# Atarilab/iterative_learning_NMPC

Hardware: AMD Instinct MI355X
Metric: MPC solves/sec (horizon-50 centroidal, batch) (higher is better)
Workload: dtype f32; 1 GPU; configs[1]: batch=1024/GPU centroidal quadruped NMPC nx=12 nu=12 N=50 fp32, 1 SQP x 6 IPM Riccati sweeps per solve, warm-start shift + solve per step; global_batch=1024, horizon=50, parallelism=dp1 (independent problems; no collective)

## Files before the change

include/nmpc.h:

```cpp
#ifndef NMPC_H
#define NMPC_H
#include <stddef.h>

#ifdef __cplusplus
extern "C" {
#endif

#define NMPC_MODEL_DOUBLE_INTEGRATOR 0
#define NMPC_MODEL_CENTROIDAL        1
#define NMPC_MODEL_WHOLEBODY         2

#define NMPC_MP_DT    0
#define NMPC_MP_MASS  1
#define NMPC_MP_IXX   2
#define NMPC_MP_IYY   3
#define NMPC_MP_IZZ   4
#define NMPC_MP_GZ    5
#define NMPC_MP_MU    6
#define NMPC_MP_UMAX  7
#define NMPC_MP_PGAIN 8
#define NMPC_MP_HIPX  9
#define NMPC_MP_HIPY  10
#define NMPC_MP_LHIP  11
#define NMPC_MP_L1    12
// ... 41 lines not shown
int nmpc_shift_warm_start(void *handle, int B, int shift, float *X, float *U, void *stream);

int nmpc_solve_batch(void *handle, int B, const float *x0, const float *yref, int yref_per_stage,
                     const float *yref_e, const float *params, float *X, float *U, int *status,
                     float *stats, void *stream);

int nmpc_shift_solve_batch(void *handle, int B, int shift, const float *x0, const float *yref,
                           int yref_per_stage, const float *yref_e, const float *params, float *X,
                           float *U, int *status, float *stats, void *stream);

int nmpc_riccati_batch(void *handle, int Bsz, int nx, int nu, const float *Q, const float *R,
                       const float *q, const float *r, const float *A, const float *B_,
                       const float *d, const float *dx0, float *dX, float *dU, int *status,
                       void *stream);

int nmpc_tracking_error(void *handle, int B, int T, int ns, const float *S, const float *S_nom,
                        float *err, float *weight, float threshold, float ood_weight, void *stream);

typedef struct {
    int n_replans;
    int nodes_per_replan;
    int replanning_steps;
    int nodes_per_cycle;
    int start_node;
    int first_solve;
    int max_sqp_first;
    float nlp_tol_first;
    float nlp_tol;
    double sim_dt, time_horizon, nom_height, height_offset;
    float push_start, push_duration;
    int footsteps;
    int record_sim_steps;
    float hip_offset[8];
    float stance_ratio[4];
    float nominal_period;
    float foot_size;
    int terminate_mask;
    float collision_height;
} nmpc_rollout_cfg;
#define NMPC_ROLLOUT_FLAG_SOLVER        1
#define NMPC_ROLLOUT_FLAG_ROLL          2
#define NMPC_ROLLOUT_FLAG_PITCH         4
#define NMPC_ROLLOUT_FLAG_HEIGHT        8
#define NMPC_ROLLOUT_FLAG_VEL_TRACKING 16
#define NMPC_ROLLOUT_FLAG_COLLISION    32
#define NMPC_ROLLOUT_FLAG_MASK       0xFF
#define NMPC_ROLLOUT_TERM_SHIFT         8
int nmpc_rollout_batch(void *handle, int B, const nmpc_rollout_cfg *cfg, const signed char *gait, float *x,
                       const double *v_des, const double *w_des, double *ref_state, float *foot_pos,
                       const float *push_force, const float *phase, float *X, float *U, float *S,
                       int *status, int *failed, void *stream);

#define NMPC_ROLLOUT_FLAG_JOINT_LIMIT   64

typedef struct {
    int n_replans;
    int replanning_steps;
    int nodes_per_cycle;
    int first_solve;
    int last_node;
    int max_sqp_first;
    float nlp_tol_first;
    float nlp_tol;
    double sim_dt, time_horizon, nom_height, height_offset;
    float step_height;
    float push_start, push_duration;
    int record_sim_steps;
    int force_reference_gravity;
    float nominal_period;
    int terminate_mask;
    float collision_height;
} nmpc_wb_rollout_cfg;
int nmpc_wb_rollout_batch(void *handle, int B, const nmpc_wb_rollout_cfg *cfg, const signed char *gait,
                          const signed char *peaks, const int *nodes, float *q, float *v, const double *v_des,
                          const double *w_des, double *ref_state, const float *joint_ref, const float *push_force,
                          float *X, float *U, float *S, int *status, int *failed, void *stream);

int nmpc_wb_rollout_set_actions(void *handle, void *torque_handle, const int *zoh, float kp, float kd, float *A);

int nmpc_set_skip(void *handle, const int *flags, int mask);

int nmpc_debug_read_tile(void *handle, int b, int k, int which, float *out_host);

int nmpc_debug_read_workspace(void *handle, int b, size_t offset, size_t count, float *out_host);
int nmpc_debug_wb_layout(int N, size_t *out8);

int nmpc_debug_set_buffer(void *handle, float *dev_buffer);

#ifdef __cplusplus
}
#endif
#endif
```

iterative_learning_nmpc_amd/_lib.py:

```python
from __future__ import annotations

import ctypes
import os
from ctypes import POINTER, c_char_p, c_float, c_int, c_size_t, c_void_p
from typing import Optional

import torch

_HERE = os.path.dirname(os.path.abspath(__file__))
LIB_PATH = os.environ.get("NMPC_HIP_LIB") or os.path.join(_HERE, "libnmpc_hip.so")

NMPC_OK = 0
NMPC_STATUS_OK, NMPC_STATUS_NAN, NMPC_STATUS_MAXITER, NMPC_STATUS_MINSTEP, NMPC_STATUS_QP = 0, 1, 2, 3, 4
STATUS_NAMES = {NMPC_STATUS_OK: "ok", NMPC_STATUS_NAN: "nan", NMPC_STATUS_MAXITER: "max_iter",
                NMPC_STATUS_MINSTEP: "min_step", NMPC_STATUS_QP: "qp_failure"}
NMPC_ROLLOUT_FLAG_SOLVER = 1
NMPC_ROLLOUT_FLAG_ROLL = 2
NMPC_ROLLOUT_FLAG_PITCH = 4
NMPC_ROLLOUT_FLAG_HEIGHT = 8
NMPC_ROLLOUT_FLAG_VEL_TRACKING = 16
NMPC_ROLLOUT_FLAG_COLLISION = 32
NMPC_ROLLOUT_FLAG_JOINT_LIMIT = 64
NMPC_ROLLOUT_FLAG_MASK = 0xFF
NMPC_ROLLOUT_TERM_SHIFT = 8

SIGNATURES = {
    "nmpc_model_dims": (c_int, [c_int, POINTER(c_int), POINTER(c_int), POINTER(c_int), POINTER(c_int)]),
    "nmpc_model_output_dims": (c_int, [c_int, POINTER(c_int), POINTER(c_int)]),
    "nmpc_create": (c_int, [c_void_p, c_int, POINTER(c_void_p)]),
    "nmpc_destroy": (None, [c_void_p]),
    "nmpc_last_error": (c_char_p, [c_void_p]),
    "nmpc_workspace_bytes": (c_size_t, [c_void_p]),
    "nmpc_set_model_params": (c_int, [c_void_p, POINTER(c_float), c_int]),
    "nmpc_set_weights": (c_int, [c_void_p, POINTER(c_float), POINTER(c_float), c_float, c_float]),
    "nmpc_set_opts": (c_int, [c_void_p, c_int, c_int, c_float, c_float, c_int]),
    "nmpc_set_contact_patterns": (c_int, [c_void_p, c_int]),
    "nmpc_set_skip": (c_int, [c_void_p, c_void_p, c_int]),
    "nmpc_wb_rollout_set_actions": (c_int, [c_void_p, c_void_p, c_void_p, c_float, c_float, c_void_p]),
    "nmpc_set_ipm": (c_int, [c_void_p, c_float, c_float, c_float, c_float, c_float, c_float]),
    "nmpc_shift_warm_start": (c_int, [c_void_p, c_int, c_int, c_void_p, c_void_p, c_void_p]),
    "nmpc_solve_batch": (c_int, [c_void_p, c_int, c_void_p, c_void_p, c_int, c_void_p, c_void_p,
                                 c_void_p, c_void_p, c_void_p, c_void_p, c_void_p]),
    "nmpc_shift_solve_batch": (c_int, [c_void_p, c_int, c_int, c_void_p, c_void_p, c_int, c_void_p, c_void_p,
                                 c_void_p, c_void_p, c_void_p, c_void_p, c_void_p]),
    "nmpc_riccati_batch": (c_int, [c_void_p, c_int, c_int, c_int] + [c_void_p] * 12),
    "nmpc_tracking_error": (c_int, [c_void_p, c_int, c_int, c_int, c_void_p, c_void_p, c_void_p,
                                    c_void_p, c_float, c_float, c_void_p]),
    "nmpc_rollout_batch": (c_int, [c_void_p, c_int, c_void_p] + [c_void_p] * 14),
    "nmpc_wb_rollout_batch": (c_int, [c_void_p, c_int, c_void_p] + [c_void_p] * 16),
    "nmpc_policy_create": (c_int, [c_void_p, c_int, POINTER(c_void_p)]),
    "nmpc_policy_destroy": (None, [c_void_p]),
    "nmpc_policy_last_error": (ctypes.c_char_p, [c_void_p]),
    "nmpc_policy_param_count": (ctypes.c_size_t, [c_void_p]),
    "nmpc_policy_set_params": (c_int, [c_void_p, c_void_p, c_void_p, c_void_p, c_void_p]),
    "nmpc_policy_get_params": (c_int, [c_void_p, c_void_p, c_void_p, c_void_p, c_void_p]),
    "nmpc_policy_forward": (c_int, [c_void_p, c_int, c_void_p, c_void_p, c_void_p]),
    "nmpc_policy_train_step": (c_int, [c_void_p, c_int, c_void_p, c_void_p, c_float, c_void_p, c_void_p, c_void_p]),
    "nmpc_weighted_sample": (c_int, [c_void_p, ctypes.c_longlong, c_int, ctypes.c_ulonglong, c_void_p, c_void_p, c_void_p]),
    "nmpc_gather_rows": (c_int, [c_void_p, ctypes.c_longlong, c_int, c_void_p, c_int, c_void_p, c_void_p]),
    "nmpc_policy_train_epoch_scratch": (ctypes.c_size_t, [ctypes.c_longlong]),
    "nmpc_policy_train_epoch": (c_int, [c_void_p, c_void_p, c_void_p, c_int, c_int, ctypes.c_ulonglong, c_float, c_void_p,
                                        c_void_p, c_void_p, c_void_p]),
    "nmpc_policy_loss": (c_int, [c_void_p, ctypes.c_longlong, c_void_p, c_void_p, c_void_p, c_void_p]),
    "nmpc_dataset_last_error": (ctypes.c_char_p, []),
    "nmpc_ring_append": (c_int, [c_void_p, c_int, ctypes.c_longlong, c_void_p, ctypes.c_longlong, ctypes.c_longlong, c_void_p]),
    "nmpc_column_stats_scratch": (ctypes.c_size_t, [c_int]),
    "nmpc_column_stats": (c_int, [c_void_p, ctypes.c_longlong, c_int, c_void_p, c_void_p, c_void_p, c_void_p]),
    "nmpc_assemble_batch": (c_int, [c_void_p, c_int, c_void_p, c_void_p, c_int, c_void_p, c_int, c_void_p, c_void_p,
                                    c_void_p, c_int, ctypes.c_longlong, c_void_p, c_int, c_void_p, c_void_p, c_void_p]),
    "nmpc_torque_create": (c_int, [c_void_p, c_int, POINTER(c_void_p)]),
    "nmpc_torque_destroy": (None, [c_void_p]),
    "nmpc_torque_last_error": (ctypes.c_char_p, [c_void_p]),
    "nmpc_id_torques_batch": (c_int, [c_void_p, c_int, c_void_p, c_void_p, c_void_p, c_void_p, c_void_p, c_void_p]),
    "nmpc_pd_torques_batch": (c_int, [c_void_p, c_int, c_void_p, c_void_p, c_void_p, c_void_p, c_void_p, c_float, c_float,
                                      c_void_p, c_void_p]),
    "nmpc_pd_target_action_batch": (c_int, [c_void_p, c_int, c_void_p, c_void_p, c_void_p, c_void_p, c_float, c_float,
                                            c_void_p, c_void_p]),
    "nmpc_plan_actions_batch": (c_int, [c_void_p, c_int, c_int, c_int, c_void_p, c_void_p, c_void_p, ctypes.c_double,
                                        ctypes.c_double, c_float, c_float, c_void_p, c_void_p, c_int, c_void_p, c_int, c_void_p]),
    "nmpc_debug_read_tile": (c_int, [c_void_p, c_int, c_int, c_int, POINTER(c_float)]),
    "nmpc_debug_set_buffer": (c_int, [c_void_p, c_void_p]),
    "nmpc_debug_read_workspace": (c_int, [c_void_p, c_int, c_size_t, c_size_t, POINTER(c_float)]),
    "nmpc_debug_wb_layout": (c_int, [c_int, POINTER(c_size_t)]),
}


class NmpcPolicyDims(ctypes.Structure):
    _fields_ = [("n_in", c_int), ("n_out", c_int), ("n_hidden", c_int), ("hidden", c_int),
                ("batch_norm", c_int), ("batch_max", c_int)]


class NmpcBatchSource(ctypes.Structure):
    _fields_ = [("states", c_void_p), ("n_state", c_int), ("s_mean", c_void_p), ("s_std", c_void_p), ("s_first", c_int),
                ("goals", c_void_p), ("n_goal", c_int), ("g_mean", c_void_p), ("g_std", c_void_p),
                ("actions", c_void_p), ("n_action", c_int), ("n_rows", ctypes.c_longlong)]


class NmpcTreeModel(ctypes.Structure):
    _fields_ = [("n_joints", c_int), ("n_actuated", c_int), ("n_feet", c_int),
                ("parent", POINTER(c_int)), ("type", POINTER(c_int)), ("axis", POINTER(c_float)),
                ("placement", POINTER(c_float)), ("mass", POINTER(c_float)), ("com", POINTER(c_float)),
                ("inertia", POINTER(c_float)), ("foot_joint", POINTER(c_int)), ("foot_offset", POINTER(c_float)),
                ("gravity", c_float * 3)]


class NmpcRolloutCfg(ctypes.Structure):
    _fields_ = [("n_replans", c_int), ("nodes_per_replan", c_int), ("replanning_steps", c_int),
                ("nodes_per_cycle", c_int), ("start_node", c_int), ("first_solve", c_int),
                ("max_sqp_first", c_int), ("nlp_tol_first", c_float), ("nlp_tol", c_float),
                ("sim_dt", ctypes.c_double), ("time_horizon", ctypes.c_double), ("nom_height", ctypes.c_double),
                ("height_offset", ctypes.c_double), ("push_start", c_float), ("push_duration", c_float),
                ("footsteps", c_int), ("record_sim_steps", c_int), ("hip_offset", c_float * 8),
                ("stance_ratio", c_float * 4), ("nominal_period", c_float), ("foot_size", c_float),
                ("terminate_mask", c_int), ("collision_height", c_float)]


class NmpcWbRolloutCfg(ctypes.Structure):
    _fields_ = [("n_replans", c_int), ("replanning_steps", c_int), ("nodes_per_cycle", c_int), ("first_solve", c_int),
                ("last_node", c_int), ("max_sqp_first", c_int), ("nlp_tol_first", c_float), ("nlp_tol", c_float),
                ("sim_dt", ctypes.c_double), ("time_horizon", ctypes.c_double), ("nom_height", ctypes.c_double),
                ("height_offset", ctypes.c_double), ("step_height", c_float), ("push_start", c_float), ("push_duration", c_float),
                ("record_sim_steps", c_int), ("force_reference_gravity", c_int), ("nominal_period", c_float),
                ("terminate_mask", c_int), ("collision_height", c_float)]


class NmpcDims(ctypes.Structure):
    _fields_ = [("model_id", c_int), ("N", c_int), ("B_max", c_int), ("precision", c_int)]


_lib = None


def load() -> ctypes.CDLL:
    global _lib
    if _lib is not None:
        return _lib
    if not os.path.exists(LIB_PATH):
        raise ImportError(
            f"{LIB_PATH} not found: build the HIP extension first "
            "(python -c 'import __graft_entry__ as g; g.build()' or iterative_learning_nmpc_amd/csrc/build.sh). "
            "This package has no CPU fallback.")
    try:
        lib = ctypes.CDLL(LIB_PATH)
    except OSError as e:
        raise ImportError(f"cannot load {LIB_PATH}: {e}") from e
    for name, (res, args) in SIGNATURES.items():
        fn = getattr(lib, name)
        fn.restype, fn.argtypes = res, args
    _lib = lib
    return lib


class NmpcError(RuntimeError):
    pass


_LAST_ERROR = {"solve": "nmpc_last_error", "policy": "nmpc_policy_last_error", "torque": "nmpc_torque_last_error",
               "dataset": "nmpc_dataset_last_error"}


def check(rc: int, handle=None, what: str = "", family: str = "solve") -> None:
    if rc != NMPC_OK:
        last_error = getattr(load(), _LAST_ERROR[family])
        msg = last_error() if family == "dataset" else last_error(handle)
        raise NmpcError(f"{what} failed ({rc}): {msg.decode() if msg else ''}")

# ... 8 lines not shown
```

iterative_learning_nmpc_amd/csrc/nmpc_api.hip:

```cpp
#include <hip/hip_runtime.h>

#include <cmath>
#include <cstdio>
#include <cstdlib>
#include <cstring>
#include <string>

#include "../../include/nmpc_torque.h"
#include "nmpc_host.hpp"
#include "nmpc_torque_plan.hpp"
#include "nmpc_solve.hip"
#include "nmpc_wb.hip"
#include "nmpc_aux.hip.inc"
#include "nmpc_rollout.hip.inc"
#include "nmpc_wb_rollout.hip.inc"

namespace {

using nmpc::fail;
using nmpc::launched;

struct Handle {
    nmpc_dims dims{};
    int device = 0;
// ... 50 lines not shown
nmpc::SolveArgs base_args(const Handle* h) {
    nmpc::SolveArgs a = handle_args<nmpc::SolveArgs>(h);
    for (int j = 0; j < 16; ++j)
        a.rs_free[j] = (j < h->nu) ? 1.0f / std::sqrt(h->W[h->nx + j] + h->reg) : 1.0f;
    a.line_search = h->line_search; a.rho = h->rho;
    a.dbg = h->dbg;
    return a;
}

template <class M>
size_t ws_floats_per_problem(int N) { return nmpc::WsLayout<M>(N).stride; }

nmpc::wb::WbArgs wb_args(const Handle* h) {
    nmpc::wb::WbArgs a = handle_args<nmpc::wb::WbArgs>(h);
    a.precision = h->dims.precision;
    a.pos_rows = h->pos_rows ? 1 : 0;
    return a;
}

int clean_workspace(Handle* h, hipStream_t st) {
    if (h->ws_dirty) {
        NMPC_TRY(h, hipMemsetAsync(h->ws, 0, h->ws_bytes, st));
        h->ws_dirty = false;
    }
    return NMPC_OK;
}

template <class A>
int launch_sqp(Handle* h, A a, hipStream_t st, size_t lds_bytes, void (*qp)(const A), void (*linearize)(const A)) {
    if (lds_bytes > 64 * 1024)
        NMPC_TRY(h, hipFuncSetAttribute(reinterpret_cast<const void*>(qp), hipFuncAttributeMaxDynamicSharedMemorySize, (int)lds_bytes));
    const long long nthreads = (long long)a.B * (a.N + 1);
    const unsigned lin_blocks = (unsigned)((nthreads + 63) / 64);
    const int shift = a.shift;
    for (int it = 0; it < a.max_sqp; ++it) {
        a.it = it;
        a.shift = (it == 0) ? shift : 0;
        if (linearize) hipLaunchKernelGGL(linearize, dim3(lin_blocks), dim3(64), 0, st, a);
        hipLaunchKernelGGL(qp, dim3(a.B), dim3(64), lds_bytes, st, a);
    }
    return launched(h);
}

int launch_wb(Handle* h, nmpc::wb::WbArgs a, hipStream_t st) {
    if (h->line_search) return fail(h, NMPC_E_ARG, "the whole-body model takes full steps (line_search = 0)");
    auto misaligned = [](const void* p, unsigned m) { return (reinterpret_cast<uintptr_t>(p) & (m - 1u)) != 0; };
    if (misaligned(a.x0, 8) || misaligned(a.yref, 8) || misaligned(a.yref_e, 8) || misaligned(a.X, 8) || misaligned(a.U, 8) || misaligned(a.params, 16))
        return fail(h, NMPC_E_ARG, "whole-body arrays must be 8 B aligned (params: 16 B)");
    return launch_sqp(h, a, st, (size_t)nmpc::wb::WbLds(a.N).total * sizeof(float), nmpc::wb::nmpc_wb_qp_kernel,
                      nmpc::wb::nmpc_wb_linearize_kernel);
}

template <class M, bool LEAN, bool BF16B, bool ALLV>
int launch_qp(Handle* h, nmpc::SolveArgs a, hipStream_t st) {
    const size_t bytes = (size_t)nmpc::Lds<M, LEAN>(a.N).total * sizeof(float);
    if (bytes > 160 * 1024) return fail(h, NMPC_E_ARG, "horizon too long for the LDS-resident layout");
    void (*const qp)(const nmpc::SolveArgs) = nmpc::nmpc_qp_kernel<M, LEAN, BF16B, ALLV>;
    void (*const linearize)(const nmpc::SolveArgs) = nmpc::nmpc_linearize_kernel<M>;
    return launch_sqp(h, a, st, bytes, qp, nmpc::qp_linearizes_itself(LEAN, a.N) ? nullptr : linearize);
}

template <class M>
int launch_solve(Handle* h, nmpc::SolveArgs a, hipStream_t st) {
    if (a.N > 64 * nmpc::N_LANE_STAGES) return fail(h, NMPC_E_ARG, "horizon too long for the lane = stage phases");
    auto in_flight = [&](size_t lds_bytes, long long per_simd) -> long long {
        if (lds_bytes > 160 * 1024) return 0;
        const long long by_lds = (long long)((160 * 1024) / lds_bytes);
        return (long long)h->n_cu * (by_lds < 4 * per_simd ? by_lds : 4 * per_simd);
    };
    const long long resident_waves = in_flight((size_t)nmpc::Lds<M, false>(a.N).total * sizeof(float), 1);
    const long long lean_waves = in_flight((size_t)nmpc::Lds<M, true>(a.N).total * sizeof(float), 2);
    const bool lean = h->force_variant ? (h->force_variant > 1)
                                       : (resident_waves == 0 || ((long long)a.B > resident_waves && lean_waves > resident_waves));
    if constexpr (M::N_STATIC_MASKS > 4) {
        if (h->all_patterns) {
            if (h->dims.precision == 1)
                return lean ? launch_qp<M, true, true, true>(h, a, st) : launch_qp<M, false, true, true>(h, a, st);
            return lean ? launch_qp<M, true, false, true>(h, a, st) : launch_qp<M, false, false, true>(h, a, st);
        }
    }
    if (h->dims.precision == 1)
        return lean ? launch_qp<M, true, true, false>(h, a, st) : launch_qp<M, false, true, false>(h, a, st);
    return lean ? launch_qp<M, true, false, false>(h, a, st) : launch_qp<M, false, false, false>(h, a, st);
}

template <class M>
int read_tile(Handle* h, int b, int k, int which, float* out) {
    using G = nmpc::TileGeom<M>;
    const nmpc::WsLayout<M> wl(h->dims.N);
    const size_t off[4] = {wl.At + (size_t)k * G::A_FLOATS, wl.Bt + (size_t)k * G::B_FLOATS,
                           wl.Kt + (size_t)k * G::K_FLOATS, wl.Ct + (size_t)k * G::C_FLOATS};
    const size_t len[4] = {G::A_FLOATS, G::B_FLOATS, G::K_FLOATS, G::C_FLOATS};
    float img[512];
    NMPC_TRY(h, hipMemcpy(img, h->ws + (size_t)b * wl.stride + off[which], len[which] * sizeof(float),
                         hipMemcpyDeviceToHost));
    std::memset(out, 0, 256 * sizeof(float));
    if (which == 0) {
        for (int c = 0; c <= M::NX; ++c)
            for (int i = 0; i < M::NX; ++i) out[i * 16 + c] = img[c * G::SA + i];
        out[M::NX * 16 + M::NX] = 1.0f;
    } else if (which == 1) {
        for (int c = 0; c < M::NU; ++c)
            for (int i = 0; i < M::NX; ++i) out[i * 16 + c] = img[c * G::SA + i];
    } else {
        const int rows = which == 2 ? M::NU : M::NX;
        for (int i = 0; i < rows; ++i) {
            for (int c = 0; c < M::NX; ++c) out[i * 16 + c] = img[i * 16 + nmpc::slot_of(c)];
            out[i * 16 + M::NX] = img[i * 16 + nmpc::HS];
        }
        if (which == 3) out[M::NX * 16 + M::NX] = 1.0f;
    }
    return NMPC_OK;
}
template <class Cfg, class R, class A, class Plan, class AfterSolve>
int run_rollout(Handle* h, int B, const Cfg* cfg, hipStream_t st, R& r, A& a, void (*prepare)(const R),
                int (*solve)(Handle*, A, hipStream_t), void (*advance)(const R), Plan plan, AfterSolve after_solve) {
    NMPC_ENTER(h, h->device);
    if (const int rc = clean_workspace(h, st)) return rc;
    const int N = h->dims.N;
    r.B = B; r.N = N; r.npc = cfg->nodes_per_cycle; r.replanning_steps = cfg->replanning_steps; r.n_replans = cfg->n_replans;
    r.record_sim_steps = cfg->record_sim_steps ? 1 : 0;
    r.sim_dt = cfg->sim_dt; r.t_horizon = cfg->time_horizon; r.nom_height = cfg->nom_height; r.height_offset = cfg->height_offset;
    r.dt_nodes = cfg->time_horizon / N;
    r.nominal_period = cfg->nominal_period; r.collision_height = cfg->collision_height;
    r.term_mask = cfg->terminate_mask & NMPC_ROLLOUT_FLAG_MASK;
    const int rows_per_replan = r.record_sim_steps ? cfg->replanning_steps : 1;
    r.n_rows = cfg->n_replans * rows_per_replan;
    a.B = B; a.yref_per_stage = 1;
    a.yref = r.yref; a.yref_e = r.yref_e; a.params = r.params; a.X = r.X; a.U = r.U; a.stats = nullptr;
    a.skip = r.term_mask ? r.failed : nullptr; a.skip_mask = r.term_mask;
    const double dt_replan = cfg->replanning_steps * cfg->sim_dt, slack = 0.5 * cfg->sim_dt;
    for (int i = 0; i < cfg->n_replans; ++i) {
        const bool cold = cfg->first_solve && i == 0;
        r.first = cold ? 1 : 0;
        r.replan_index = i;
        r.row0 = i * rows_per_replan;
        const double t_now = i * dt_replan;
        r.push_dt = (r.push_force && cfg->push_duration > 0.0f && t_now >= (double)cfg->push_start - slack &&
                     t_now < (double)cfg->push_start + (double)cfg->push_duration - slack) ? (float)dt_replan : 0.0f;
        const int shift = plan(i);
        hipLaunchKernelGGL(prepare, dim3(B), dim3(64), 0, st, r);
        a.shift = cold ? 0 : (shift > N ? N : shift);
        a.max_sqp = cold ? cfg->max_sqp_first : h->max_sqp;
        a.nlp_tol = cold ? cfg->nlp_tol_first : cfg->nlp_tol;
        if (const int rc = solve(h, a, st)) return rc;
        if (const int rc = after_solve(i)) return rc;
        hipLaunchKernelGGL(advance, dim3((B + 63) / 64), dim3(64), 0, st, r);
    }
    return launched(h);
}

int allocate(Handle* h) {
    NMPC_TRY(no_handle, hipDeviceGetAttribute(&h->n_cu, hipDeviceAttributeMultiprocessorCount, h->device));
    NMPC_TRY(no_handle, hipMalloc(reinterpret_cast<void**>(&h->ws), h->ws_bytes));
    NMPC_TRY(no_handle, hipMemset(h->ws, 0, h->ws_bytes));
    const int N = h->dims.N;
    const size_t per = (size_t)N * h->ny + h->nye + (size_t)(N + 1) * (h->np > 0 ? h->np : 1) + h->nx;
    NMPC_TRY(no_handle, hipMalloc(reinterpret_cast<void**>(&h->roll), ((size_t)h->dims.B_max * per + 16) * sizeof(float)));
    return NMPC_OK;
}
}

extern "C" {

int nmpc_model_dims(int model_id, int* nx, int* nu, int* np, int* ng) {
    int d[4];
// ... 299 lines not shown
    if (B == 0) return NMPC_OK;
    if (!cfg || !gait || !peaks || !nodes || !q || !v || !v_des || !w_des || !ref_state || !joint_ref || !X || !U || !S || !status || !failed)
        return fail(h, NMPC_E_ARG, "null argument");
    if (h->dims.model_id != NMPC_MODEL_WHOLEBODY) return fail(h, NMPC_E_ARG, "nmpc_wb_rollout_batch needs the whole-body model");
    if (const int rc = check_batch(h, B)) return rc;
    if (cfg->n_replans < 1 || cfg->replanning_steps < 1 || cfg->nodes_per_cycle < 1 || !(cfg->sim_dt > 0) || !(cfg->time_horizon > 0))
        return fail(h, NMPC_E_ARG, "rollout configuration out of range");
    if (const int rc = check_configured(h)) return rc;
    if (h->line_search) return fail(h, NMPC_E_ARG, "the whole-body model takes full steps (line_search = 0)");
    const int N = h->dims.N;
    if (cfg->replanning_steps * cfg->sim_dt > cfg->time_horizon) return fail(h, NMPC_E_ARG, "replanning interval longer than the horizon");
    for (int i = 0; i < cfg->n_replans; ++i)
        if (nodes[i] < 0 || (i > 0 && nodes[i] < nodes[i - 1])) return fail(h, NMPC_E_ARG, "nodes must be non-negative and non-decreasing");
    const auto& lab = h->labels;
    if (lab.A) {
        if (!cfg->record_sim_steps) return fail(h, NMPC_E_ARG, "action labels go with rows per simulation step: record_sim_steps must be 1");
        if (const char* why = nmpc_torque::plan_actions_refusal(lab.torque, cfg->replanning_steps, lab.zoh, lab.kp, h->device))
            return fail(h, NMPC_E_ARG, std::string("action labels: ") + why);
    }
    hipStream_t st = static_cast<hipStream_t>(stream);
    auto up4 = [](size_t n) { return (n + 3) & ~(size_t)3; };
    nmpc::wb::WbRolloutArgs r{};
    r.yref = h->roll;
    r.yref_e = r.yref + up4((size_t)h->dims.B_max * N * h->ny);
    r.params = r.yref_e + up4((size_t)h->dims.B_max * h->nye);
    r.x0 = r.params + up4((size_t)h->dims.B_max * (N + 1) * h->np);
    r.force_gravity = cfg->force_reference_gravity ? 1 : 0;
    r.step_height = cfg->step_height;
    r.mp = h->mp;
    r.gait = gait; r.peaks = peaks; r.q = q; r.v = v; r.v_des = v_des; r.w_des = w_des; r.ref_state = ref_state;
    r.joint_ref = joint_ref; r.push_force = push_force;
    r.X = X; r.U = U; r.S = S; r.status = status; r.failed = failed;
    nmpc::wb::WbArgs w = wb_args(h);
    w.x0 = r.x0; w.status = status;
    int last_node = cfg->last_node;
    return run_rollout(h, B, cfg, st, r, w, nmpc::wb::nmpc_wb_rollout_prepare_kernel, launch_wb, nmpc::wb::nmpc_wb_rollout_advance_kernel,
                       [&](int i) {
                           const int shift = nodes[i] - last_node;
                           r.node = last_node = nodes[i];
                           return shift;
                       },
                       [&](int) {
                           if (!lab.A) return (int)NMPC_OK;
                           const int steps = cfg->replanning_steps;
                           const int lrc = nmpc_plan_actions_batch(lab.torque, B, steps, N, X, U, lab.zoh, r.dt_nodes, r.sim_dt, lab.kp, lab.kd, nullptr,
                                                                   r.term_mask ? failed : nullptr, r.term_mask, lab.A + (size_t)r.row0 * 12, r.n_rows, st);
                           if (lrc) return fail(h, lrc, std::string("nmpc_plan_actions_batch: ") + nmpc_torque_last_error(lab.torque));
                           if (r.term_mask)
                               hipLaunchKernelGGL(nmpc::wb::nmpc_wb_rollout_hold_actions_kernel, dim3((unsigned)(((size_t)B * steps * 12 + 255) / 256)),
                                                  dim3(256), 0, st, B, r.n_rows, r.row0, steps, r.term_mask, failed, lab.A);
                           return (int)NMPC_OK;
                       });
}

int nmpc_debug_set_buffer(void* handle, float* dev_buffer) {
    Handle* h = static_cast<Handle*>(handle);
    if (!h) return NMPC_E_ARG;
    h->dbg = dev_buffer;
    return NMPC_OK;
}

int nmpc_debug_read_tile(void* handle, int b, int k, int which, float* out_host) {
    Handle* h = static_cast<Handle*>(handle);
    if (!h || !out_host) return fail(h, NMPC_E_ARG, "null argument");
    if (b < 0 || b >= h->dims.B_max || k < 0 || k >= h->dims.N || which < 0 || which > 3)
        return fail(h, NMPC_E_ARG, "index out of range");
    NMPC_ENTER(h, h->device);
    NMPC_TRY(h, hipDeviceSynchronize());
    if (h->dims.model_id == NMPC_MODEL_DOUBLE_INTEGRATOR) return read_tile<nmpc::DoubleIntegrator>(h, b, k, which, out_host);
    if (h->dims.model_id == NMPC_MODEL_WHOLEBODY) return fail(h, NMPC_E_ARG, "use nmpc_debug_read_workspace for the whole-body model");
    return read_tile<nmpc::Centroidal>(h, b, k, which, out_host);
}

int nmpc_debug_read_workspace(void* handle, int b, size_t offset, size_t count, float* out_host) {
    Handle* h = static_cast<Handle*>(handle);
    if (!h || !out_host) return fail(h, NMPC_E_ARG, "null argument");
    if (b < 0 || b >= h->dims.B_max || offset + count > h->ws_stride) return fail(h, NMPC_E_ARG, "index out of range");
    NMPC_ENTER(h, h->device);
    NMPC_TRY(h, hipDeviceSynchronize());
    NMPC_TRY(h, hipMemcpy(out_host, h->ws + (size_t)b * h->ws_stride + offset, count * sizeof(float), hipMemcpyDeviceToHost));
    return NMPC_OK;
}

int nmpc_debug_wb_layout(int N, size_t* out8) {
    if (!out8 || N < 1) return NMPC_E_ARG;
    const nmpc::wb::WsLayout wl(N);
    const nmpc::wb::StageArr sa(N);
    out8[0] = wl.rec; out8[1] = wl.js; out8[2] = wl.qt; out8[3] = wl.kt; out8[4] = wl.arr; out8[5] = wl.stride;
    out8[6] = (size_t)sa.NS; out8[7] = (size_t)nmpc::wb::REC;
    return NMPC_OK;
}

}
```

iterative_learning_nmpc_amd/csrc/nmpc_solve.hip:

```cpp
#include <hip/hip_runtime.h>

#include <type_traits>

#include "../../include/nmpc.h"
#include "nmpc_models.hpp"
#include "nmpc_sweep.hpp"

namespace nmpc {

struct SolveArgs {
    ModelParams mp;
    float W[32];
    float rs_free[16];
    float We[16];
    float reg, reg_e;
    int N, B;
    int max_sqp, n_ipm, line_search, yref_per_stage;
    int it;
    int shift;
    float nlp_tol, mu0, sigma, s_min, gamma, tau_min, rho;
    const float* x0;
    const float* yref;
    const float* yref_e;
    const float* params;
    float* X;
    float* U;
    int* status;
    float* stats;
    float* ws;
    float* dbg;
    const int* skip;
    int skip_mask;
};

__device__ __forceinline__ bool skipped(const SolveArgs& a, int b) { return a.skip && (a.skip[b] & a.skip_mask) != 0; }

__host__ __device__ inline int round4(int n) { return (n + 3) & ~3; }

__device__ __forceinline__ int shifted_node(int k, int shift, int N) {
    return (k >= 1 && k <= N - shift) ? k + shift : k;
}
__device__ __forceinline__ bool shifted_stage_valid(int k, int shift, int N) { return k < N - shift; }

template <class M>
struct TileGeom {
    static_assert(M::NX <= 12 && M::NU <= 12, "slot layout: at most 12 states and 12 inputs");
    static constexpr int SA = (M::NX + 3) & ~3;
    static constexpr int RQ = SA / 4;
    static constexpr int KQ = (M::NU + 2) / 3;
    static constexpr int CQ = (M::NX + 2) / 3;
    static constexpr int A_FLOATS = (((M::NX + 1) * SA) + 31) & ~31;
    static constexpr int B_FLOATS = ((M::NU * SA) + 31) & ~31;
    static constexpr int K_FLOATS = ((3 * KQ * TS) + 31) & ~31;
    static constexpr int C_FLOATS = ((3 * CQ * TS) + 31) & ~31;
};

typedef float f32x3u __attribute__((ext_vector_type(3), aligned(4)));

template <class M>
struct ImageLane {
    using G = TileGeom<M>;
    unsigned a_off, b_off, t_off;
    bool a_ok, b_ok, t_ok;
    __device__ __forceinline__ void init(int lane) {
        const int q = lane >> 4, c = lane & 15;
        const int jc = (c == HS) ? M::NX : index_of(c);
        a_ok = (jc >= 0) && (jc <= M::NX) && (3 * q < M::NX);
        b_ok = (index_of(c) >= 0) && (index_of(c) < M::NU) && (3 * q < M::NX);
        a_off = 4u * ((a_ok ? jc : 0) * G::SA + (a_ok ? 3 * q : 0));
        b_off = 4u * ((b_ok ? index_of(c) : 0) * G::SA + (b_ok ? 3 * q : 0));
        t_ok = (index_of(c) >= 0) && (index_of(c) < M::NX) && (3 * q < M::NU);
        t_off = 4u * ((t_ok ? 3 * q : 0) * G::SA + (t_ok ? index_of(c) : 0));
    }
    __device__ __forceinline__ f32x4 load3(const float* img, unsigned off) const {
        const f32x3u v = *reinterpret_cast<const f32x3u*>(reinterpret_cast<const char*>(img) + (size_t)off);
        return f32x4{v[0], v[1], v[2], 0.0f};
    }
    __device__ __forceinline__ f32x4 load_A(const float* img) const { return load3(img, a_off); }
    __device__ __forceinline__ f32x4 load_B(const float* img) const { return load3(img, b_off); }
    __device__ __forceinline__ f32x4 load_Bt(const float* img) const {
        f32x4 o;
#pragma unroll
        for (int r = 0; r < 3; ++r) o[r] = ld_f32(img, t_off, 4 * r * G::SA);
        o[3] = 0.0f;
        return o;
    }
    __device__ __forceinline__ f32x4 fix_A(f32x4 v, int lane) const {
        const int q = lane >> 4, c = lane & 15;
        f32x4 o;
#pragma unroll
        for (int r = 0; r < 3; ++r) o[r] = (a_ok && 3 * q + r < M::NX) ? v[r] : 0.0f;
        o[3] = (q == 0 && c == HS) ? 1.0f : 0.0f;
        return o;
    }
    __device__ __forceinline__ f32x4 fix_B(f32x4 v, int lane) const {
        const int q = lane >> 4;
        f32x4 o;
#pragma unroll
        for (int r = 0; r < 3; ++r) o[r] = (b_ok && 3 * q + r < M::NX) ? v[r] : 0.0f;
        o[3] = 0.0f;
        return o;
    }
    __device__ __forceinline__ f32x4 fix_Bt(f32x4 v, int lane) const {
        const int q = lane >> 4;
        f32x4 o;
#pragma unroll
        for (int r = 0; r < 3; ++r) o[r] = (t_ok && 3 * q + r < M::NU) ? v[r] : 0.0f;
        o[3] = 0.0f;
        return o;
    }
};
struct RowStoreLane {
    unsigned off, step;
    __device__ __forceinline__ void init(int lane, int nq, int image_floats, int k_first, int k_scratch) {
        const int q = lane >> 4, c = lane & 15;
        const bool valid = q < nq;
        off = 4u * ((valid ? k_first : k_scratch) * image_floats + (valid ? 3 * q * TS : 0) + c);
        step = valid ? 4u * image_floats : 0u;
    }
    __device__ __forceinline__ void store(float* images, f32x4 v) {
#pragma unroll
        for (int r = 0; r < 3; ++r) st_f32(images, off, 4 * r * TS, v[r]);
        off -= step;
    }
};

template <class M>
struct StageArrays {
    int NS;
    int nX, nU, nG;
    int Xs, Us, dX, dU, dXp, dUp, sv, lv, total;
    __host__ __device__ StageArrays(int N, bool stage_major) {
        NS = (N + 1) | 1;
        nX = stage_major ? (N + 1) * TS : M::NX * NS;
        nU = stage_major ? (N + 1) * TS : M::NU * NS;
        nG = stage_major ? (N + 1) * TS : M::NG * NS;
        int o = 0;
        Xs = o;  o += round4(nX);
        Us = o;  o += round4(nU);
        dX = o;  o += round4(nX);
        dU = o;  o += round4(nU);
        dXp = o; o += round4(nX);
        dUp = o; o += round4(nU);
        sv = o;  o += round4(nG);
        lv = o;  o += round4(nG);
        o += 4;
        total = o;
    }
};

template <class M>
struct WsLayout {
    size_t At, Bt, Kt, Ct, q, r, c, act, umk, cost, flag, lean, stride;
    __host__ __device__ explicit WsLayout(int N) {
        size_t o = 0;
        At = o; o += (size_t)N * TileGeom<M>::A_FLOATS;
        Bt = o; o += (size_t)N * TileGeom<M>::B_FLOATS;
        Kt = o; o += (size_t)(N + 1) * TileGeom<M>::K_FLOATS;
        Ct = o; o += (size_t)(N + 1) * TileGeom<M>::C_FLOATS;
        q = o; o += round4((N + 1) * M::NX);
        r = o; o += round4(N * M::NU);
        c = o; o += round4(N * M::NG);
        act = o; o += round4(N);
        umk = o; o += round4(N);
        cost = o; o += round4(N + 1);
        flag = o; o += 4;
        lean = o; o += StageArrays<M>(N, true).total;
        stride = (o + 63) & ~(size_t)63;
    }
};
constexpr int N_LANE_STAGES = 4;
__host__ __device__ constexpr bool qp_linearizes_itself(bool lean, int N) { return lean && N < 64; }

#ifdef NMPC_STAMPS
#define STAMP_DECL unsigned long long st_t0 = __builtin_readcyclecounter(), st_acc[8] = {0, 0, 0, 0, 0, 0, 0, 0}; \
    StageStamps sst = {0, {0, 0, 0, 0, 0, 0, 0, 0}}
#define SST_PASS , sst
#define SST_TILES(i) SST(i)
#define STAMP(i) do { const unsigned long long st_t1 = __builtin_readcyclecounter(); st_acc[i] += st_t1 - st_t0; st_t0 = st_t1; } while (0)
#else
#define STAMP_DECL
#define STAMP(i)
#define SST_PASS
#define SST_TILES(i)
#endif

template <class M, bool LEAN>
struct Lds {
    int arr, qv, rv, gsq, gvt, act, umk, runs, conv, dx0, total;
    __host__ __device__ explicit Lds(int N) {
        const int NS = (N + 1) | 1;
        int o = 0;
// ... 439 lines not shown
                    }
                }
                phase_sync();
            }
            STAMP(1);
            f32x4 P;
            {
                const float qc = c_is_x ? qv[N * TS + c] : 0.0f;
#pragma unroll
                for (int r = 0; r < 4; ++r) {
                    const int row = 4 * q4 + r, ir = index_of(row);
                    const bool r_is_x = ir >= 0 && ir < NX;
                    float v = 0.0f;
                    if (row == c && r_is_x) v = we_c;
                    if (c == HS && r_is_x) v = qv[N * TS + row];
                    if (row == HS && c_is_x) v = qc;
                    P[r] = v;
                }
            }
            auto sweep = [&](auto ipm_tag) {
                constexpr bool IPM = decltype(ipm_tag)::value;
                struct NextCost {
                    f32x4 Gs, Vt, Tb, Qn, Sn, Rn;
                    const float *qrow, *rrow, *sqrow, *vtrow;
                    const float* qcol;
                    const bool *qm, *rm;
                    f32x4 Qc, Rc, Gc;
                    bool hx_col;
                    f32x4 q4v, r4v, sq4, vt4;
                    float qcv;
                    __device__ __forceinline__ void fetch() {
                        q4v = *reinterpret_cast<const f32x4*>(qrow);
                        r4v = *reinterpret_cast<const f32x4*>(rrow);
                        qcv = *qcol;
                        if constexpr (IPM) {
                            sq4 = *reinterpret_cast<const f32x4*>(sqrow);
                            vt4 = *reinterpret_cast<const f32x4*>(vtrow);
                        }
                    }
                    __device__ __forceinline__ void build() {
                        Rn = Rc;
#pragma unroll
                        for (int r = 0; r < 4; ++r) {
                            Qn[r] = Qc[r] + (qm[r] ? (hx_col ? q4v[r] : qcv) : 0.0f);
                            Sn[r] = rm[r] ? r4v[r] : 0.0f;
                        }
                        if constexpr (IPM) {
#pragma unroll
                            for (int r = 0; r < 4; ++r) {
                                Gs[r] = Gc[r] * sq4[r];
                                Vt[r] = hx_col ? vt4[r] : Gs[r];
                            }
                            Tb = zero4();
                        }
                    }
                    __device__ __forceinline__ void mfma(int i) {
                        if constexpr (IPM && !BF16B) Tb = __builtin_amdgcn_mfma_f32_16x16x4f32(Gs[i], Vt[i], Tb, 0, 0, 0);
                        if constexpr (IPM && BF16B) { if (i == 0) Tb = xty_bf16(Gs, Vt); }
                    }
                    __device__ __forceinline__ void finish() {
                        if constexpr (IPM) {
#pragma unroll
                            for (int r = 0; r < 4; ++r) {
                                Rn[r] += hx_col ? 0.0f : Tb[r];
                                Sn[r] += hx_col ? Tb[r] : 0.0f;
                            }
                        }
                    }
                };
                auto next_cost = [&](int kk) {
                    NextCost nc;
                    nc.qrow = qv + kk * TS + 4 * q4; nc.rrow = rv + kk * TS + 4 * q4;
                    nc.sqrow = gsq + kk * TS + 4 * q4; nc.vtrow = gvt + kk * TS + 4 * q4;
                    nc.qcol = qv + kk * TS + c;
                    nc.qm = qm; nc.rm = rm;
                    nc.Qc = Qc; nc.Rc = Rc; nc.Gc = Gc; nc.hx_col = is_hx_col;
                    return nc;
                };
                ImageLane<M> il;
                il.init(lane);
                RowStoreLane ks, cs;
                ks.init(lane, G::KQ, G::K_FLOATS, N - 1, N);
                cs.init(lane, G::CQ, G::C_FLOATS, N - 1, N);
                f32x4 A0 = il.fix_A(il.load_A(At + (size_t)(N - 1) * G::A_FLOATS), lane);
                f32x4 B0 = il.fix_B(il.load_B(Bt + (size_t)(N - 1) * G::B_FLOATS), lane);
                f32x4 T0 = il.fix_Bt(il.load_Bt(Bt + (size_t)(N - 1) * G::B_FLOATS), lane);
                f32x4 Qt, St, Rt;
                {
                    NextCost nc = next_cost(N - 1);
                    nc.fetch();
                    nc.build();
#pragma unroll
                    for (int i = 0; i < 4; ++i) nc.mfma(i);
                    nc.finish();
                    Qt = nc.Qn; St = nc.Sn; Rt = nc.Rn;
                }
                int lane_zero = 0;
                asm volatile("" : "+v"(lane_zero));
                if constexpr (LEAN) {
                    unsigned cm = umask[N - 1];
                    for (int k = N - 1; k >= 0; --k) {
    #ifdef NMPC_STAMPS
                        sst.t0 = __builtin_readcyclecounter();
    #endif
                        const int kn = (k > 0) ? k - 1 : 0;
    #ifdef QP_T_ONEIMG
                        const int ki = (a.B < 0) ? kn : 0;
    #else
                        const int ki = kn;
    #endif
                        const f32x4 A1 = il.load_A(At + (size_t)ki * G::A_FLOATS);
                        const f32x4 B1 = il.load_B(Bt + (size_t)ki * G::B_FLOATS);
                        const f32x4 T1 = il.load_Bt(Bt + (size_t)ki * G::B_FLOATS);
                        const unsigned cm_next = umask[kn + lane_zero];
                        f32x4 Kk, Acl;
                        NextCost sh = next_cost(kn);
                        auto run = [&](auto mask_tag) {
                            constexpr unsigned MK = decltype(mask_tag)::value;
                            constexpr unsigned STEPS = (IPM && !BF16B && MK != DYNAMIC_MASK) ? M::barrier_steps(MK) : 0xFu;
                            return backward_stage<NU, MK, true, ALLV, STEPS, LEAN ? 0 : 2>(P, A0, B0, T0, Qt, St, Rt, conv, sl, lane,
                                                                            cm & 0xFFFFu, Kk, Acl, sh SST_PASS);
                        };
                        bool ok = true;
    #define NMPC_VARIANT(I)                                                                                   \
        case I:                                                                                               \
            if constexpr (I < M::N_STATIC_MASKS)                                                              \
                ok = run(std::integral_constant<unsigned, M::static_mask(I < M::N_STATIC_MASKS ? I : 0)>{}); \
            else ok = run(std::integral_constant<unsigned, DYNAMIC_MASK>{});                                  \
            break;
    #define NMPC_COMMON(J) (M::common_variant(J) >= 0 && vi == M::common_variant(J))
    #define NMPC_RUN_COMMON(J) run(std::integral_constant<unsigned, M::static_mask(M::common_variant(J) >= 0 ? M::common_variant(J) : 0)>{})
                        const int vi = ((cm >> 24) & 1u) ? WIDEST : (int)((cm >> 16) & 0x1Fu) - 1;
                        if constexpr (!ALLV) {
                            if (NMPC_COMMON(0)) ok = NMPC_RUN_COMMON(0);
                            else if (NMPC_COMMON(1)) ok = NMPC_RUN_COMMON(1);
                            else if (NMPC_COMMON(2)) ok = NMPC_RUN_COMMON(2);
                            else if (NMPC_COMMON(3)) ok = NMPC_RUN_COMMON(3);
                            else ok = run(std::integral_constant<unsigned, DYNAMIC_MASK>{});
                        } else {
                            switch (vi) {
                                NMPC_VARIANT(0) NMPC_VARIANT(1) NMPC_VARIANT(2) NMPC_VARIANT(3)
                                NMPC_VARIANT(4) NMPC_VARIANT(5) NMPC_VARIANT(6) NMPC_VARIANT(7)
                                NMPC_VARIANT(8) NMPC_VARIANT(9) NMPC_VARIANT(10) NMPC_VARIANT(11)
                                NMPC_VARIANT(12) NMPC_VARIANT(13) NMPC_VARIANT(14) NMPC_VARIANT(15)
                                default: ok = run(std::integral_constant<unsigned, DYNAMIC_MASK>{});
                            }
                        }
    #undef NMPC_VARIANT
    #undef NMPC_COMMON
    #undef NMPC_RUN_COMMON
                        qp_ok = ok && qp_ok;
    #ifdef QP_T_NOSTORE
                        if (a.B < 0)
    #endif
                        {
                        ks.store(Kt, Kk);
                        cs.store(Ct, Acl);
                        }
                        A0 = il.fix_A(A1, lane);
                        B0 = il.fix_B(B1, lane);
                        T0 = il.fix_Bt(T1, lane);
                        Qt = sh.Qn; St = sh.Sn; Rt = sh.Rn;
                        cm = __builtin_amdgcn_readfirstlane(cm_next);
                        SST_TILES(5);
                    }
                } else {
                    auto run_stages = [&](auto mask_tag, int top, int len) {
                        constexpr unsigned MK = decltype(mask_tag)::value;
                        constexpr bool DYN = (MK == DYNAMIC_MASK);
                        constexpr unsigned STEPS = (IPM && !BF16B && !DYN) ? M::barrier_steps(MK) : 0xFu;
                        unsigned cm = 0u;
                        if constexpr (DYN) cm = __builtin_amdgcn_readfirstlane(umask[top - 1]);
                        for (int k = top - 1; k >= top - len; --k) {
#ifdef NMPC_STAMPS
                            sst.t0 = __builtin_readcyclecounter();
#endif
                            const int kn = (k > 0) ? k - 1 : 0;
#ifdef QP_T_ONEIMG
                            const int ki = (a.B < 0) ? kn : 0;
#else
                            const int ki = kn;
#endif
                            const f32x4 A1 = il.load_A(At + (size_t)ki * G::A_FLOATS);
                            const f32x4 B1 = il.load_B(Bt + (size_t)ki * G::B_FLOATS);
                            const f32x4 T1 = il.load_Bt(Bt + (size_t)ki * G::B_FLOATS);
                            unsigned cm_next = 0u;
                            if constexpr (DYN) cm_next = umask[kn + lane_zero];
                            f32x4 Kk, Acl;
                            NextCost sh = next_cost(kn);
                            const bool ok = backward_stage<NU, MK, true, ALLV, STEPS, LEAN ? 0 : 2>(P, A0, B0, T0, Qt, St, Rt, conv, sl, lane,
                                                                                                 cm & 0xFFFFu, Kk, Acl, sh SST_PASS);
                            qp_ok = ok && qp_ok;
#ifdef QP_T_NOSTORE
                            if (a.B < 0)
#endif
                            {
                            ks.store(Kt, Kk);
                            cs.store(Ct, Acl);
                            }
                            A0 = il.fix_A(A1, lane);
                            B0 = il.fix_B(B1, lane);
                            T0 = il.fix_Bt(T1, lane);
                            Qt = sh.Qn; St = sh.Sn; Rt = sh.Rn;
                            if constexpr (DYN) cm = __builtin_amdgcn_readfirstlane(cm_next);
                            SST_TILES(5);
                        }
                    };
#define NMPC_VARIANT(I)                                                                                                 \
        case I:                                                                                                             \
            if constexpr (I < M::N_STATIC_MASKS)                                                                            \
                run_stages(std::integral_constant<unsigned, M::static_mask(I < M::N_STATIC_MASKS ? I : 0)>{}, top, len);    \
            else run_stages(std::integral_constant<unsigned, DYNAMIC_MASK>{}, top, len);                                    \
            break;
#define NMPC_COMMON(J) (M::common_variant(J) >= 0 && key == J##u)
#define NMPC_RUN_COMMON(J) run_stages(std::integral_constant<unsigned, M::static_mask(M::common_variant(J) >= 0 ? M::common_variant(J) : 0)>{}, top, len)
                    unsigned rw = __builtin_amdgcn_readfirstlane(runs[0]);
                    for (int r = 1; (rw & 0x1FFu) != 0u; ++r) {
                        const unsigned rw_next = runs[r + lane_zero];
                        const int top = (int)(rw & 0x1FFu), len = (int)((rw >> 9) & 0x1FFu);
                        const unsigned key = rw >> 18;
                        if constexpr (!ALLV) {
                            if (NMPC_COMMON(0)) NMPC_RUN_COMMON(0);
                            else if (NMPC_COMMON(1)) NMPC_RUN_COMMON(1);
                            else if (NMPC_COMMON(2)) NMPC_RUN_COMMON(2);
                            else if (NMPC_COMMON(3)) NMPC_RUN_COMMON(3);
                            else run_stages(std::integral_constant<unsigned, DYNAMIC_MASK>{}, top, len);
                        } else {
                            switch (key) {
                                NMPC_VARIANT(0) NMPC_VARIANT(1) NMPC_VARIANT(2) NMPC_VARIANT(3)
                                NMPC_VARIANT(4) NMPC_VARIANT(5) NMPC_VARIANT(6) NMPC_VARIANT(7)
                                NMPC_VARIANT(8) NMPC_VARIANT(9) NMPC_VARIANT(10) NMPC_VARIANT(11)
                                NMPC_VARIANT(12) NMPC_VARIANT(13) NMPC_VARIANT(14) NMPC_VARIANT(15)
                                default: run_stages(std::integral_constant<unsigned, DYNAMIC_MASK>{}, top, len);
                            }
                        }
                        rw = __builtin_amdgcn_readfirstlane(rw_next);
                    }
#undef NMPC_VARIANT
#undef NMPC_COMMON
#undef NMPC_RUN_COMMON
                }
            };
            if (use_ipm) sweep(std::true_type{}); else sweep(std::false_type{});
            __threadfence_block();
            wave_sync();
            STAMP(2);
            float* oX = use_ipm ? dXp : dX;
            float* oU = use_ipm ? dUp : dU;
            float vs[NX];
            if constexpr (LEAN) {
#pragma unroll
                for (int i = 0; i < NX; ++i) vs[i] = dx0s[i];
                if (lane < NX) AT(oX, 0, lane) = dx0s[lane];
            } else {
#pragma unroll
                for (int i = 0; i < NX; ++i) vs[i] = x0[i] - AT(Xs, 0, i);
                if (lane < NX) AT(oX, 0, lane) = x0[lane] - AT(Xs, 0, lane);
            }
            constexpr int FWD_PF = 4, RQ4 = slot_of(NX - 1) / 4 + 1;
            const bool is_x = lane < NX, is_u = (lane >= 16 && lane < 16 + NU);
            unsigned rowoff = 4u * (unsigned)((is_x ? wl.Ct : wl.Kt) + (is_x ? lane : is_u ? lane - 16 : 0) * TS);
            const unsigned rowstep = 4u * (is_x ? G::C_FLOATS : G::K_FLOATS);
            float* dst = is_x ? &AT(oX, 1, lane) : is_u ? &AT(oU, 0, lane - 16) : idle_sink;
            const int dstep = (is_x || is_u) ? (LEAN ? TS : 1) : 0;
            auto load_row = [&](unsigned off, f32x4 (&row)[RQ4]) {
                row[0] = *reinterpret_cast<const f32x4*>(reinterpret_cast<const char*>(ws) + (size_t)off);
#pragma unroll
                for (int g = 1; g < RQ4; ++g) {
                    const f32x3u v = *reinterpret_cast<const f32x3u*>(reinterpret_cast<const char*>(ws) + (size_t)off + 16 * g);
                    row[g] = f32x4{v[0], v[1], v[2], 0.0f};
                }
            };
            f32x4 ring[FWD_PF][RQ4];
#pragma unroll
            for (int j = 0; j < FWD_PF; ++j) load_row(rowoff + (unsigned)((j < N) ? j : N - 1) * rowstep, ring[j]);
            const unsigned rowlast = rowoff + (unsigned)(N - 1) * rowstep;
            rowoff += FWD_PF * rowstep;
            auto fwd_stage = [&](int k, f32x4 (&slot)[RQ4]) {
                float acc = slot[0][HS], acc1 = 0.0f, acc2 = 0.0f, acc3 = 0.0f;
#pragma unroll
                for (int i = 0; i < NX; ++i) {
                    const float e = slot[slot_of(i) >> 2][slot_of(i) & 3];
                    float& ac = (i & 3) == 0 ? acc : (i & 3) == 1 ? acc1 : (i & 3) == 2 ? acc2 : acc3;
                    asm volatile("v_fmac_f32 %0, %1, %2" : "+v"(ac) : "s"(vs[i]), "v"(e));
                }
                acc = (acc + acc1) + (acc2 + acc3);
#ifdef QP_T_ONEIMG
                load_row((a.B < 0) ? rowoff : rowlast, slot);
// ... 274 lines not shown
```

Measured before the change: 2.418 million solves/s.

## Pad tile images with zero slots so masked lanes load zeros, skip fixups

```diff
diff --git a/include/nmpc.h b/include/nmpc.h
--- a/include/nmpc.h
+++ b/include/nmpc.h
@@ -147,6 +147,8 @@
 
 int nmpc_debug_read_tile(void *handle, int b, int k, int which, float *out_host);
 
+int nmpc_debug_image_geometry(int model_id, int *out8, unsigned *lane_floats);
+
 int nmpc_debug_read_workspace(void *handle, int b, size_t offset, size_t count, float *out_host);
 int nmpc_debug_wb_layout(int N, size_t *out8);
 
diff --git a/iterative_learning_nmpc_amd/_lib.py b/iterative_learning_nmpc_amd/_lib.py
--- a/iterative_learning_nmpc_amd/_lib.py
+++ b/iterative_learning_nmpc_amd/_lib.py
@@ -82,6 +82,7 @@
     "nmpc_debug_set_buffer": (c_int, [c_void_p, c_void_p]),
     "nmpc_debug_read_workspace": (c_int, [c_void_p, c_int, c_size_t, c_size_t, POINTER(c_float)]),
     "nmpc_debug_wb_layout": (c_int, [c_int, POINTER(c_size_t)]),
+    "nmpc_debug_image_geometry": (c_int, [c_int, POINTER(c_int), POINTER(ctypes.c_uint)]),
 }
 
 
diff --git a/iterative_learning_nmpc_amd/csrc/nmpc_api.hip b/iterative_learning_nmpc_amd/csrc/nmpc_api.hip
--- a/iterative_learning_nmpc_amd/csrc/nmpc_api.hip
+++ b/iterative_learning_nmpc_amd/csrc/nmpc_api.hip
@@ -156,6 +156,20 @@
     if (h->dims.precision == 1)
         return lean ? launch_qp<M, true, true, false>(h, a, st) : launch_qp<M, false, true, false>(h, a, st);
     return lean ? launch_qp<M, true, false, false>(h, a, st) : launch_qp<M, false, false, false>(h, a, st);
+}
+
+template <class M>
+void image_geometry(int* out8, unsigned* lane_floats) {
+    using G = nmpc::TileGeom<M>;
+    const int g[8] = {M::NX, M::NU, G::SA, G::A_FLOATS, G::B_FLOATS, G::A_ZERO, G::B_ZERO, 0};
+    for (int i = 0; i < 8; ++i) out8[i] = g[i];
+    for (int lane = 0; lane < 64; ++lane) {
+        nmpc::ImageLane<M> il;
+        il.init(lane);
+        lane_floats[3 * lane + 0] = il.a_off / 4u;
+        lane_floats[3 * lane + 1] = il.b_off / 4u;
+        lane_floats[3 * lane + 2] = il.t_off / 4u;
+    }
 }
 
 template <class M>
@@ -621,6 +635,14 @@
     return NMPC_OK;
 }
 
+int nmpc_debug_image_geometry(int model_id, int* out8, unsigned* lane_floats) {
+    if (!out8 || !lane_floats) return NMPC_E_ARG;
+    if (model_id == NMPC_MODEL_DOUBLE_INTEGRATOR) image_geometry<nmpc::DoubleIntegrator>(out8, lane_floats);
+    else if (model_id == NMPC_MODEL_CENTROIDAL) image_geometry<nmpc::Centroidal>(out8, lane_floats);
+    else return NMPC_E_ARG;
+    return NMPC_OK;
+}
+
 int nmpc_debug_wb_layout(int N, size_t* out8) {
     if (!out8 || N < 1) return NMPC_E_ARG;
     const nmpc::wb::WsLayout wl(N);
diff --git a/iterative_learning_nmpc_amd/csrc/nmpc_solve.hip b/iterative_learning_nmpc_amd/csrc/nmpc_solve.hip
--- a/iterative_learning_nmpc_amd/csrc/nmpc_solve.hip
+++ b/iterative_learning_nmpc_amd/csrc/nmpc_solve.hip
@@ -49,8 +49,10 @@
     static constexpr int RQ = SA / 4;
     static constexpr int KQ = (M::NU + 2) / 3;
     static constexpr int CQ = (M::NX + 2) / 3;
-    static constexpr int A_FLOATS = (((M::NX + 1) * SA) + 31) & ~31;
-    static constexpr int B_FLOATS = ((M::NU * SA) + 31) & ~31;
+    static constexpr int A_ZERO = (M::NX + 1) * SA;
+    static constexpr int B_ZERO = M::NU * SA;
+    static constexpr int A_FLOATS = (A_ZERO + 3 + 31) & ~31;
+    static constexpr int B_FLOATS = (B_ZERO + 2 * SA + 3 + 31) & ~31;
     static constexpr int K_FLOATS = ((3 * KQ * TS) + 31) & ~31;
     static constexpr int C_FLOATS = ((3 * CQ * TS) + 31) & ~31;
 };
@@ -62,15 +64,17 @@
     using G = TileGeom<M>;
     unsigned a_off, b_off, t_off;
     bool a_ok, b_ok, t_ok;
-    __device__ __forceinline__ void init(int lane) {
+    float a_hs;
+    __host__ __device__ __forceinline__ void init(int lane) {
         const int q = lane >> 4, c = lane & 15;
         const int jc = (c == HS) ? M::NX : index_of(c);
         a_ok = (jc >= 0) && (jc <= M::NX) && (3 * q < M::NX);
         b_ok = (index_of(c) >= 0) && (index_of(c) < M::NU) && (3 * q < M::NX);
-        a_off = 4u * ((a_ok ? jc : 0) * G::SA + (a_ok ? 3 * q : 0));
-        b_off = 4u * ((b_ok ? index_of(c) : 0) * G::SA + (b_ok ? 3 * q : 0));
+        a_off = 4u * (a_ok ? jc * G::SA + 3 * q : G::A_ZERO);
+        b_off = 4u * (b_ok ? index_of(c) * G::SA + 3 * q : G::B_ZERO);
         t_ok = (index_of(c) >= 0) && (index_of(c) < M::NX) && (3 * q < M::NU);
-        t_off = 4u * ((t_ok ? 3 * q : 0) * G::SA + (t_ok ? index_of(c) : 0));
+        t_off = 4u * (t_ok ? 3 * q * G::SA + index_of(c) : G::B_ZERO);
+        a_hs = (q == 0 && c == HS) ? 1.0f : 0.0f;
     }
     __device__ __forceinline__ f32x4 load3(const float* img, unsigned off) const {
         const f32x3u v = *reinterpret_cast<const f32x3u*>(reinterpret_cast<const char*>(img) + (size_t)off);
@@ -108,6 +112,18 @@
         for (int r = 0; r < 3; ++r) o[r] = (t_ok && 3 * q + r < M::NU) ? v[r] : 0.0f;
         o[3] = 0.0f;
         return o;
+    }
+    __device__ __forceinline__ f32x4 tile_A(f32x4 v, int lane) const {
+        if constexpr (M::NX % 3 != 0) return fix_A(v, lane);
+        else return f32x4{v[0], v[1], v[2], a_hs};
+    }
+    __device__ __forceinline__ f32x4 tile_B(f32x4 v, int lane) const {
+        if constexpr (M::NX % 3 != 0) return fix_B(v, lane);
+        else return v;
+    }
+    __device__ __forceinline__ f32x4 tile_Bt(f32x4 v, int lane) const {
+        if constexpr (M::NU % 3 != 0) return fix_Bt(v, lane);
+        else return v;
     }
 };
 struct RowStoreLane {
@@ -713,9 +729,10 @@
                 RowStoreLane ks, cs;
                 ks.init(lane, G::KQ, G::K_FLOATS, N - 1, N);
                 cs.init(lane, G::CQ, G::C_FLOATS, N - 1, N);
-                f32x4 A0 = il.fix_A(il.load_A(At + (size_t)(N - 1) * G::A_FLOATS), lane);
-                f32x4 B0 = il.fix_B(il.load_B(Bt + (size_t)(N - 1) * G::B_FLOATS), lane);
-                f32x4 T0 = il.fix_Bt(il.load_Bt(Bt + (size_t)(N - 1) * G::B_FLOATS), lane);
+                f32x4 A0 = il.load_A(At + (size_t)(N - 1) * G::A_FLOATS);
+                f32x4 B0 = il.load_B(Bt + (size_t)(N - 1) * G::B_FLOATS);
+                f32x4 T0 = il.load_Bt(Bt + (size_t)(N - 1) * G::B_FLOATS);
+                if constexpr (LEAN) { A0 = il.fix_A(A0, lane); B0 = il.fix_B(B0, lane); T0 = il.fix_Bt(T0, lane); }
                 f32x4 Qt, St, Rt;
                 {
                     NextCost nc = next_cost(N - 1);
@@ -796,13 +813,15 @@
                         SST_TILES(5);
                     }
                 } else {
+                    f32x4 A1, B1, T1;
                     auto run_stages = [&](auto mask_tag, int top, int len) {
                         constexpr unsigned MK = decltype(mask_tag)::value;
                         constexpr bool DYN = (MK == DYNAMIC_MASK);
                         constexpr unsigned STEPS = (IPM && !BF16B && !DYN) ? M::barrier_steps(MK) : 0xFu;
                         unsigned cm = 0u;
                         if constexpr (DYN) cm = __builtin_amdgcn_readfirstlane(umask[top - 1]);
-                        for (int k = top - 1; k >= top - len; --k) {
+                        auto stage = [&](int k, const f32x4& Ac, const f32x4& Bc, const f32x4& Tc, f32x4& An, f32x4& Bn, f32x4& Tn)
+                                         __attribute__((always_inline)) {
 #ifdef NMPC_STAMPS
                             sst.t0 = __builtin_readcyclecounter();
 #endif
@@ -812,14 +831,15 @@
 #else
                             const int ki = kn;
 #endif
-                            const f32x4 A1 = il.load_A(At + (size_t)ki * G::A_FLOATS);
-                            const f32x4 B1 = il.load_B(Bt + (size_t)ki * G::B_FLOATS);
-                            const f32x4 T1 = il.load_Bt(Bt + (size_t)ki * G::B_FLOATS);
+                            An = il.load_A(At + (size_t)ki * G::A_FLOATS);
+                            Bn = il.load_B(Bt + (size_t)ki * G::B_FLOATS);
+                            Tn = il.load_Bt(Bt + (size_t)ki * G::B_FLOATS);
                             unsigned cm_next = 0u;
                             if constexpr (DYN) cm_next = umask[kn + lane_zero];
                             f32x4 Kk, Acl;
                             NextCost sh = next_cost(kn);
-                            const bool ok = backward_stage<NU, MK, true, ALLV, STEPS, LEAN ? 0 : 2>(P, A0, B0, T0, Qt, St, Rt, conv, sl, lane,
+                            const bool ok = backward_stage<NU, MK, true, ALLV, STEPS, LEAN ? 0 : 2>(P, il.tile_A(Ac, lane), il.tile_B(Bc, lane),
+                                                                                                 il.tile_Bt(Tc, lane), Qt, St, Rt, conv, sl, lane,
                                                                                                  cm & 0xFFFFu, Kk, Acl, sh SST_PASS);
                             qp_ok = ok && qp_ok;
 #ifdef QP_T_NOSTORE
@@ -829,12 +849,25 @@
                             ks.store(Kt, Kk);
                             cs.store(Ct, Acl);
                             }
-                            A0 = il.fix_A(A1, lane);
-                            B0 = il.fix_B(B1, lane);
-                            T0 = il.fix_Bt(T1, lane);
                             Qt = sh.Qn; St = sh.Sn; Rt = sh.Rn;
                             if constexpr (DYN) cm = __builtin_amdgcn_readfirstlane(cm_next);
                             SST_TILES(5);
+                        };
+                        int k = top - 1;
+                        if constexpr (!ALLV) {
+                            for (int pairs = len >> 1; pairs > 0; --pairs, k -= 2) {
+                                stage(k, A0, B0, T0, A1, B1, T1);
+                                stage(k - 1, A1, B1, T1, A0, B0, T0);
+                            }
+                            if (len & 1) {
+                                stage(k, A0, B0, T0, A1, B1, T1);
+                                A0 = A1; B0 = B1; T0 = T1;
+                            }
+                        } else {
+                            for (; k >= top - len; --k) {
+                                stage(k, A0, B0, T0, A1, B1, T1);
+                                A0 = A1; B0 = B1; T0 = T1;
+                            }
                         }
                     };
 #define NMPC_VARIANT(I)                                                                                                 \
```

Result: no change. 2.409 million solves/s (-0.4%).
